# microsoft/fadtk

Hardware: NVIDIA H100
Metric: audio_seconds_embedded_per_second (higher is better)
Workload: dtype f16

## Files before the change

fadtk_b200/csrc/conv_gemm.cuh:

```cuda
#pragma once
#include "sm90.cuh"

namespace fad {

struct ConvGemmParams {
    int taps;
    int cblks;
    int box_w, box_h, box_n;
    int tiles_w, tiles_h;
    int img_groups;
    int n_tiles;
    int H, W, NB, Cout;
    int lo_adds;
    int ld_out, n_valid;
    int relu, pool;
    const float* bias;
    __half* out;
    float* out_f32;
    float* resid;
    int resid_C, resid_res, resid_shift;
};

__device__ __forceinline__ long long window_row_to_token(long long o, int res, int shift) {
    const int lg_nw = 28 - __clz(res);
    const int nw = res >> 3;
    const int in = (int)(o & 63);
    const long long wi = o >> 6;
    const int wx = (int)wi & (nw - 1);
    const int wy = (int)(wi >> lg_nw) & (nw - 1);
    const long long b = wi >> (2 * lg_nw);
    int y = wy * 8 + (in >> 3) + shift, xx = wx * 8 + (in & 7) + shift;
    if (y >= res) y -= res;
    if (xx >= res) xx -= res;
    return (b * res + y) * res + xx;
}

constexpr int kTileM = 128;
constexpr int kBlockK = 64;
constexpr int kConvGemmThreads = 384;
constexpr int kConsumers = 2;
constexpr int kClusterCtas = 2;
constexpr int kChunkSteps = 8;
constexpr float kAccumShrinkPerElement = 1.06e-9f;
constexpr uint32_t kABytes = kTileM * kBlockK * 2;
constexpr uint32_t kEpiRowBytes = 128 * 4;
constexpr uint32_t kEpiBytes = 64 * kEpiRowBytes;
constexpr uint32_t kStagingBytes = 32 * 128;

template <int N_TILE, int WMODE>
__host__ __device__ constexpr uint32_t conv_gemm_stage_bytes() {
    return kABytes + (WMODE == 1 ? 2 : 1) * N_TILE * kBlockK * 2;
}

template <int N_TILE, int STAGES, int WMODE>
__host__ __device__ constexpr uint32_t conv_gemm_smem_bytes() {
    return STAGES * conv_gemm_stage_bytes<N_TILE, WMODE>() + 1024  + 256
         + kConsumers * kEpiBytes;
}

__device__ __forceinline__ uint32_t pack_half2(float a, float b) {
    __half2 h = __floats2half2_rn(a, b);
    return *reinterpret_cast<uint32_t*>(&h);
}
__device__ __forceinline__ float gelu_erf(float x) {
    const float z = fminf(fabsf(x) * 0.70710678118654752f, 4.3f);
    float q = 1.04899843e-04f;
    q = fmaf(q, z, -4.92790774e-04f);
    q = fmaf(q, z, -2.22368206e-03f);
    q = fmaf(q, z, 2.93586859e-02f);
    q = fmaf(q, z, -1.48908889e-01f);
    q = fmaf(q, z, -9.18342944e-01f);
    q = fmaf(q, z, -1.62791250e+00f);
    float e;
    asm("ex2.approx.ftz.f32 %0, %1;" : "=f"(e) : "f"(q * z));
    return 0.5f * x * (1.0f + copysignf(1.0f - e, x));
}

__device__ __forceinline__ float elu_ex2(float x) {
    float e;
    asm("ex2.approx.ftz.f32 %0, %1;" : "=f"(e) : "f"(fminf(x, 0.f) * 1.4426950408889634f));
    const float t = x * fmaf(x, fmaf(x, fmaf(x, 4.16666667e-2f, 1.66666667e-1f), 0.5f), 1.0f);
    return x > 0.f ? x : (x > -0.0625f ? t : e - 1.0f);
}

__device__ __forceinline__ uint32_t hmax2_u32(uint32_t a, uint32_t b) {
    __half2 r = __hmax2(*reinterpret_cast<__half2*>(&a), *reinterpret_cast<__half2*>(&b));
    return *reinterpret_cast<uint32_t*>(&r);
}

template <int N_TILE, int STAGES, int WMODE>
__global__ void __launch_bounds__(kConvGemmThreads, 1)
conv_gemm_kernel(const __grid_constant__ CUtensorMap map_x,
                 const __grid_constant__ CUtensorMap map_w,
                 const ConvGemmParams p)
{
    using namespace sm90;
    static_assert(N_TILE == 128, "one m64n128 accumulator per consumer warpgroup");
    static_assert(WMODE == 0 || WMODE == 1, "WMODE 0: fp16 weights, 1: fp16 hi/lo pair");
    static_assert(kClusterCtas == 2, "the work units below are M-tile pairs");
    constexpr bool SPLIT_W = WMODE == 1;
    constexpr uint32_t kStageBytes = conv_gemm_stage_bytes<N_TILE, WMODE>();
    constexpr int kBRows = (SPLIT_W ? 2 : 1) * N_TILE;
    constexpr int kColsPerThread = N_TILE / 2;
    constexpr int kGroups = kColsPerThread / 32;

    extern __shared__ uint8_t smem_raw[];
    uint8_t* smem = reinterpret_cast<uint8_t*>((reinterpret_cast<uintptr_t>(smem_raw) + 1023) & ~uintptr_t(1023));
    uint64_t* bars = reinterpret_cast<uint64_t*>(smem + STAGES * kStageBytes);
    uint64_t* full = bars;
    uint64_t* empty = bars + STAGES;
    uint8_t* epi = smem + STAGES * kStageBytes + 256;

    const int warp = threadIdx.x >> 5;
    const int lane = threadIdx.x & 31;
    const int ksteps = p.taps * p.cblks;
    const int n_chunks = (ksteps + kChunkSteps - 1) / kChunkSteps;
    const int chunk_len = (ksteps + n_chunks - 1) / n_chunks;
    const int m_tiles = p.img_groups * p.tiles_h * p.tiles_w;
    const int rank = (int)cluster_ctarank();
    const int cluster = (int)blockIdx.x / kClusterCtas;
    const int n_clusters = (int)gridDim.x / kClusterCtas;
    const int total_units = (m_tiles + 1) / 2 * p.n_tiles;

    if (warp == 0 && lane == 0) {
        tma_prefetch_desc(&map_x);
        tma_prefetch_desc(&map_w);
    }
    if (warp == 1 && lane == 0) {
        for (int s = 0; s < STAGES; ++s) { mbar_init(&full[s], 1); mbar_init(&empty[s], kClusterCtas * kConsumers * 4); }
        mbar_fence_init();
    }
    cluster_sync();

    if (warp < 4) {
        setmaxnreg_dec<40>();
        if (warp == 0 && elect_one()) {
            constexpr int kHalfRows = kBRows / kClusterCtas;
            uint8_t* const w_half = smem + kABytes + rank * kHalfRows * 128;
            int s = 0; uint32_t ph = 0;
            for (int unit = cluster; unit < total_units; unit += n_clusters) {
                const int nt = unit % p.n_tiles;
                const int m = min(2 * (unit / p.n_tiles) + rank, m_tiles - 1);
                const int w0 = (m % p.tiles_w) * p.box_w;
                const int h0 = ((m / p.tiles_w) % p.tiles_h) * p.box_h;
                const int n0 = (m / (p.tiles_w * p.tiles_h)) * p.box_n;
                for (int ks = 0; ks < ksteps; ++ks) {
                    const int tap = ks / p.cblks;
                    const int cb = ks - tap * p.cblks;
                    int dh = 0, dw = 0;
                    if (p.taps == 9) { dh = tap / 3 - 1; dw = tap % 3 - 1; }
                    mbar_wait(&empty[s], ph ^ 1);
                    uint8_t* st = smem + s * kStageBytes;
                    mbar_expect_tx(&full[s], kStageBytes);
                    tma_load_4d(st, &map_x, &full[s], cb * kBlockK, w0 + dw, h0 + dh, n0);
                    tma_load_2d_multicast(w_half + s * kStageBytes, &map_w, &full[s], ks * kBlockK,
                                          nt * kBRows + rank * kHalfRows, (1u << kClusterCtas) - 1);
                    if (++s == STAGES) { s = 0; ph ^= 1; }
                }
            }
        }
    } else {
        setmaxnreg_inc<232>();
        const int c = (warp >> 2) - 1;
        const int wg_t = threadIdx.x & 127;
        const int wq = wg_t >> 5;
        const int rr = wg_t & 63;
        const int half = wg_t >> 6;
        const int r = c * 64 + rr;
        const int bw = p.box_w, bh = p.box_h;
        const int pw = r % bw;
        const int phh = (r / bw) % bh;
        const int pn = r / (bw * bh);
        const uint32_t epi_base = smem_u32(epi) + c * kEpiBytes;
        const uint32_t bar_id = 1 + c;
        int s = 0; uint32_t ph = 0;
        const bool plain = p.tiles_w == 1 && p.tiles_h == 1 && bw == 1 && bh == 1;
        auto prefetch_resid = [&](int nt_, int m_) {
            if (p.resid == nullptr || !plain) return;
            const int n_ = m_ * kTileM + r;
            if (n_ >= p.NB) return;
            const long long tok = p.resid_res ? window_row_to_token((long long)n_, p.resid_res, p.resid_shift) : (long long)n_;
            const int c0 = nt_ * N_TILE + half * kColsPerThread;
            for (int cc = c0; cc < c0 + kColsPerThread && cc < p.resid_C; cc += 32)
                asm volatile("prefetch.global.L2 [%0];" :: "l"(p.resid + tok * p.resid_C + cc));
        };
        if (cluster < total_units) prefetch_resid(cluster % p.n_tiles, 2 * (cluster / p.n_tiles) + rank);
        auto load_bias = [&](float4 (&b)[8], int col0) {
            const float4* src = reinterpret_cast<const float4*>(p.bias + col0);
#pragma unroll
            for (int j = 0; j < 8; ++j) b[j] = __ldg(src + j);
        };
        auto release = [&](int st_) {
            __syncwarp();
            if (lane == 0) {
#pragma unroll
                for (int cta = 0; cta < kClusterCtas; ++cta) mbar_arrive_cluster(&empty[st_], cta);
            }
        };

        for (int unit = cluster; unit < total_units; unit += n_clusters) {
            const int nt = unit % p.n_tiles;
            const int m = 2 * (unit / p.n_tiles) + rank;
            if (unit + n_clusters < total_units)
                prefetch_resid((unit + n_clusters) % p.n_tiles, 2 * ((unit + n_clusters) / p.n_tiles) + rank);

            float sum[64], acc[64];
#pragma unroll
            for (int i = 0; i < 64; ++i) sum[i] = 0.f;
            for (int ks0 = 0; ks0 < ksteps; ks0 += chunk_len) {
                const int ks1 = min(ks0 + chunk_len, ksteps);
                const float unshrink = kAccumShrinkPerElement * (float)((ks1 - ks0) * kBlockK * (SPLIT_W && p.lo_adds ? 2 : 1));
                int prev_s = -1;
                for (int ks = ks0; ks < ks1; ++ks) {
                    mbar_wait(&full[s], ph);
                    const uint32_t a_addr = smem_u32(smem + s * kStageBytes);
                    const uint64_t a_desc = kmajor_sw128_desc(a_addr + c * 64 * 128);
                    const uint64_t b_desc = kmajor_sw128_desc(a_addr + kABytes);
                    wgmma_fence();
#pragma unroll
                    for (int k = 0; k < kBlockK / 16; ++k) {
                        wgmma_m64n128k16_f16<0, 0>(acc, a_desc + 2 * k, b_desc + 2 * k, (ks > ks0) || (k > 0));
                        if (SPLIT_W)
                            wgmma_m64n128k16_f16<0, 0>(acc, a_desc + 2 * k, b_desc + 2 * k + (N_TILE * 128 / 16), 1);
                    }
                    wgmma_commit();
                    wgmma_wait<1>();
                    if (prev_s >= 0) release(prev_s);
                    prev_s = s;
                    if (++s == STAGES) { s = 0; ph ^= 1; }
                }
                wgmma_wait<0>();
                fence_regs(acc);
                release(prev_s);
#pragma unroll
                for (int i = 0; i < 64; ++i) sum[i] += fmaf(acc[i], unshrink, acc[i]);
            }

            named_bar_sync(bar_id, 128);
            {
                const int fr = wq * 16 + (lane >> 2);
#pragma unroll
                for (int j = 0; j < 16; ++j) {
#pragma unroll
                    for (int i = 0; i < 2; ++i) {
                        const int row = fr + 8 * i, col = 8 * j + 2 * (lane & 3);
                        const uint32_t addr = epi_base + row * kEpiRowBytes + ((((col >> 2) ^ (row & 7))) << 4) + (col & 3) * 4;
                        sts64(addr, sum[4 * j + 2 * i], sum[4 * j + 2 * i + 1]);
                    }
                }
            }
            named_bar_sync(bar_id, 128);
            float accr[kColsPerThread];
#pragma unroll
            for (int q4 = 0; q4 < kColsPerThread / 4; ++q4) {
                const int ch = half * (kColsPerThread / 4) + q4;
                const uint4 u = lds128(epi_base + rr * kEpiRowBytes + ((ch ^ (rr & 7)) << 4));
                accr[4 * q4 + 0] = __uint_as_float(u.x); accr[4 * q4 + 1] = __uint_as_float(u.y);
                accr[4 * q4 + 2] = __uint_as_float(u.z); accr[4 * q4 + 3] = __uint_as_float(u.w);
            }
            named_bar_sync(bar_id, 128);

            int w, h, n;
            if (plain) { w = 0; h = 0; n = m * kTileM + r; }
            else {
                w = (m % p.tiles_w) * bw + pw;
                h = ((m / p.tiles_w) % p.tiles_h) * bh + phh;
                n = (m / (p.tiles_w * p.tiles_h)) * p.box_n + pn;
            }
            const bool valid = n < p.NB;
            const int ch0 = nt * N_TILE + half * kColsPerThread;
            long long out_off = -1, res_off = -1;
            if (valid && !p.pool) {
                out_off = (long long)((size_t(n) * p.H + h) * p.W + w) * p.ld_out;
                if (p.resid != nullptr)
                    res_off = (p.resid_res ? window_row_to_token((long long)n, p.resid_res, p.resid_shift) : (long long)n)
                              * p.resid_C;
            }
            const uint32_t stg = epi_base + wq * kStagingBytes;
            const uint32_t stg_mine = stg + lane * 128;
            const int sw = lane & 7;
            const int cq = lane & 7, rq = lane >> 3;
            const bool f32_path = p.out_f32 != nullptr || p.resid != nullptr;
            float4 bnext[8];
#pragma unroll
            for (int g = 0; g < kGroups; ++g) {
                float f[32];
                load_bias(bnext, ch0 + g * 32);
#pragma unroll
                for (int j = 0; j < 8; ++j) {
                    const float4 b = bnext[j];
                    f[4 * j + 0] = accr[g * 32 + 4 * j + 0] + b.x;
                    f[4 * j + 1] = accr[g * 32 + 4 * j + 1] + b.y;
                    f[4 * j + 2] = accr[g * 32 + 4 * j + 2] + b.z;
                    f[4 * j + 3] = accr[g * 32 + 4 * j + 3] + b.w;
                }
                if (p.relu == 1) {
#pragma unroll
                    for (int j = 0; j < 32; ++j) f[j] = fmaxf(f[j], 0.0f);
                } else if (p.relu == 2) {
#pragma unroll
                    for (int j = 0; j < 32; ++j) f[j] = gelu_erf(f[j]);
                } else if (p.relu == 3) {
#pragma unroll
                    for (int j = 0; j < 32; ++j) f[j] = elu_ex2(f[j]);
                }
                uint32_t h2[16];
#pragma unroll
                for (int j = 0; j < 16; ++j) h2[j] = pack_half2(f[2 * j], f[2 * j + 1]);

                if (!p.pool) {
                    if (f32_path) {
#pragma unroll
                        for (int j = 0; j < 8; ++j)
                            sts128(stg_mine + ((j ^ sw) << 4), __float_as_uint(f[4 * j]), __float_as_uint(f[4 * j + 1]),
                                   __float_as_uint(f[4 * j + 2]), __float_as_uint(f[4 * j + 3]));
                        __syncwarp();
                        float4 v[8];
#pragma unroll
                        for (int it = 0; it < 8; ++it) {
                            const int rr = it * 4 + rq;
                            const uint4 u = lds128(stg + rr * 128 + ((cq ^ (rr & 7)) << 4));
                            v[it] = make_float4(__uint_as_float(u.x), __uint_as_float(u.y), __uint_as_float(u.z), __uint_as_float(u.w));
                        }
                        const int col = ch0 + g * 32 + cq * 4;
                        if (p.out_f32 != nullptr) {
#pragma unroll
                            for (int it = 0; it < 8; ++it) {
                                const long long off = __shfl_sync(0xffffffffu, out_off, it * 4 + rq);
                                if (off >= 0 && col < p.n_valid) *reinterpret_cast<float4*>(p.out_f32 + off + col) = v[it];
                            }
                        }
                        if (p.resid != nullptr && ch0 + g * 32 < p.resid_C) {
#pragma unroll
                            for (int hf = 0; hf < 2; ++hf) {
                                long long offs[4];
                                float4 xv[4];
#pragma unroll
                                for (int it = 0; it < 4; ++it) {
                                    offs[it] = __shfl_sync(0xffffffffu, res_off, (hf * 4 + it) * 4 + rq);
                                    if (offs[it] >= 0) xv[it] = *reinterpret_cast<const float4*>(p.resid + offs[it] + col);
                                }
#pragma unroll
                                for (int it = 0; it < 4; ++it) {
                                    if (offs[it] >= 0) {
                                        const float4 a = v[hf * 4 + it];
                                        xv[it].x += a.x; xv[it].y += a.y; xv[it].z += a.z; xv[it].w += a.w;
                                        *reinterpret_cast<float4*>(p.resid + offs[it] + col) = xv[it];
                                    }
                                }
                            }
                        }
                        __syncwarp();
                        if (p.out != nullptr && out_off >= 0) {
                            uint4* dst = reinterpret_cast<uint4*>(p.out + out_off + ch0 + g * 32);
#pragma unroll
                            for (int j = 0; j < 4; ++j)
                                if (ch0 + g * 32 + 8 * j < p.n_valid)
                                    dst[j] = make_uint4(h2[4 * j], h2[4 * j + 1], h2[4 * j + 2], h2[4 * j + 3]);
                        }
                    } else if (p.out != nullptr) {
#pragma unroll
                        for (int j = 0; j < 4; ++j)
                            sts128(stg_mine + ((((g & 1) * 4 + j) ^ sw) << 4), h2[4 * j], h2[4 * j + 1], h2[4 * j + 2], h2[4 * j + 3]);
                        if (g & 1) {
                            __syncwarp();
                            const int col = ch0 + (g - 1) * 32 + cq * 8;
#pragma unroll
                            for (int it = 0; it < 8; ++it) {
                                const int rr = it * 4 + rq;
                                const uint4 v = lds128(stg + rr * 128 + ((cq ^ (rr & 7)) << 4));
                                const long long off = __shfl_sync(0xffffffffu, out_off, rr);
                                if (off >= 0 && col < p.n_valid) *reinterpret_cast<uint4*>(p.out + off + col) = v;
                            }
                            __syncwarp();
                        }
                    }
                } else {
#pragma unroll
                    for (int j = 0; j < 16; ++j) {
                        uint32_t o = __shfl_xor_sync(0xffffffffu, h2[j], 1);
                        h2[j] = hmax2_u32(h2[j], o);
                        o = __shfl_xor_sync(0xffffffffu, h2[j], bw);
                        h2[j] = hmax2_u32(h2[j], o);
                    }
                    const int sub = (pw & 1) | ((phh & 1) << 1);
                    uint4 o;
                    o.x = sub == 0 ? h2[0] : sub == 1 ? h2[4] : sub == 2 ? h2[8]  : h2[12];
                    o.y = sub == 0 ? h2[1] : sub == 1 ? h2[5] : sub == 2 ? h2[9]  : h2[13];
                    o.z = sub == 0 ? h2[2] : sub == 1 ? h2[6] : sub == 2 ? h2[10] : h2[14];
                    o.w = sub == 0 ? h2[3] : sub == 1 ? h2[7] : sub == 2 ? h2[11] : h2[15];
                    if (valid) {
                        const size_t pix = (size_t(n) * (p.H >> 1) + (h >> 1)) * (p.W >> 1) + (w >> 1);
                        *reinterpret_cast<uint4*>(p.out + pix * p.Cout + ch0 + g * 32 + sub * 8) = o;
                    }
                }
            }
        }
    }
    cluster_sync();
}

}
```

fadtk_b200/csrc/sm90.cuh:

```cuda
#pragma once
#include <cuda.h>
#include <cuda_fp16.h>
#include <stdint.h>
#include <stdio.h>

namespace sm90 {

__device__ __forceinline__ uint32_t smem_u32(const void* p) {
    return static_cast<uint32_t>(__cvta_generic_to_shared(p));
}
__device__ __forceinline__ uint32_t lane_id() { return threadIdx.x & 31; }

__device__ __forceinline__ bool elect_one() {
    uint32_t pred;
    asm volatile(
        "{\n\t.reg .pred P;\n\t"
        "elect.sync _|P, 0xffffffff;\n\t"
        "selp.u32 %0, 1, 0, P;\n\t}\n"
        : "=r"(pred));
    return pred != 0;
}

template <uint32_t kRegs> __device__ __forceinline__ void setmaxnreg_inc() {
    asm volatile("setmaxnreg.inc.sync.aligned.u32 %0;" ::"n"(kRegs));
}
template <uint32_t kRegs> __device__ __forceinline__ void setmaxnreg_dec() {
    asm volatile("setmaxnreg.dec.sync.aligned.u32 %0;" ::"n"(kRegs));
}

__device__ __forceinline__ void named_bar_sync(uint32_t id, uint32_t count) {
    asm volatile("bar.sync %0, %1;" ::"r"(id), "r"(count) : "memory");
}

__device__ __forceinline__ void sts128(uint32_t addr, uint32_t x, uint32_t y, uint32_t z, uint32_t w) {
    asm volatile("st.shared.v4.b32 [%0], {%1, %2, %3, %4};" ::"r"(addr), "r"(x), "r"(y), "r"(z), "r"(w) : "memory");
}
__device__ __forceinline__ uint4 lds128(uint32_t addr) {
    uint4 v;
    asm volatile("ld.shared.v4.b32 {%0, %1, %2, %3}, [%4];" : "=r"(v.x), "=r"(v.y), "=r"(v.z), "=r"(v.w) : "r"(addr) : "memory");
    return v;
}
__device__ __forceinline__ void sts64(uint32_t addr, float x, float y) {
    asm volatile("st.shared.v2.f32 [%0], {%1, %2};" ::"r"(addr), "f"(x), "f"(y) : "memory");
}

__device__ __forceinline__ void mbar_init(uint64_t* bar, uint32_t count) {
    asm volatile("mbarrier.init.shared::cta.b64 [%0], %1;" ::"r"(smem_u32(bar)), "r"(count));
}
__device__ __forceinline__ void mbar_fence_init() {
    asm volatile("fence.mbarrier_init.release.cluster;" ::: "memory");
}
__device__ __forceinline__ void mbar_expect_tx(uint64_t* bar, uint32_t bytes) {
    asm volatile("mbarrier.arrive.expect_tx.shared::cta.b64 _, [%0], %1;"
                 ::"r"(smem_u32(bar)), "r"(bytes) : "memory");
}
__device__ __forceinline__ void mbar_arrive(uint64_t* bar) {
    asm volatile("mbarrier.arrive.shared::cta.b64 _, [%0];" ::"r"(smem_u32(bar)) : "memory");
}
__device__ __forceinline__ bool mbar_try_wait(uint64_t* bar, uint32_t parity) {
    uint32_t ok;
    asm volatile(
        "{\n\t.reg .pred P;\n\t"
        "mbarrier.try_wait.parity.shared::cta.b64 P, [%1], %2;\n\t"
        "selp.u32 %0, 1, 0, P;\n\t}\n"
        : "=r"(ok) : "r"(smem_u32(bar)), "r"(parity) : "memory");
    return ok != 0;
}
__device__ __forceinline__ bool mbar_try_wait_hint(uint64_t* bar, uint32_t parity, uint32_t ns) {
    uint32_t ok;
    asm volatile(
        "{\n\t.reg .pred P;\n\t"
        "mbarrier.try_wait.parity.shared::cta.b64 P, [%1], %2, %3;\n\t"
        "selp.u32 %0, 1, 0, P;\n\t}\n"
        : "=r"(ok) : "r"(smem_u32(bar)), "r"(parity), "r"(ns) : "memory");
    return ok != 0;
}
__device__ __forceinline__ void mbar_wait(uint64_t* bar, uint32_t parity) {
    if (mbar_try_wait(bar, parity)) return;
    uint32_t spins = 0;
    while (!mbar_try_wait_hint(bar, parity, 2000u)) {
        if (++spins > (1u << 24)) asm volatile("trap;");
    }
}

__device__ __forceinline__ uint32_t cluster_ctarank() {
    uint32_t r;
    asm volatile("mov.u32 %0, %%cluster_ctarank;" : "=r"(r));
    return r;
}
__device__ __forceinline__ void cluster_sync() {
    asm volatile("barrier.cluster.arrive.release;\n\tbarrier.cluster.wait.acquire;" ::: "memory");
}
__device__ __forceinline__ void mbar_arrive_cluster(uint64_t* bar, uint32_t cta) {
    asm volatile(
        "{\n\t.reg .b32 ra;\n\t"
        "mapa.shared::cluster.u32 ra, %0, %1;\n\t"
        "mbarrier.arrive.shared::cluster.b64 _, [ra];\n\t}\n"
        ::"r"(smem_u32(bar)), "r"(cta) : "memory");
}

__device__ __forceinline__ void fence_proxy_async_smem() {
    asm volatile("fence.proxy.async.shared::cta;" ::: "memory");
}

__device__ __forceinline__ void tma_prefetch_desc(const CUtensorMap* m) {
    asm volatile("prefetch.tensormap [%0];" ::"l"(reinterpret_cast<uint64_t>(m)) : "memory");
}
__device__ __forceinline__ void tma_load_2d(void* dst, const CUtensorMap* m, uint64_t* bar,
                                            int c0, int c1) {
    asm volatile(
        "cp.async.bulk.tensor.2d.shared::cluster.global.mbarrier::complete_tx::bytes"
        " [%0], [%1, {%3, %4}], [%2];"
        ::"r"(smem_u32(dst)), "l"(reinterpret_cast<uint64_t>(m)), "r"(smem_u32(bar)),
          "r"(c0), "r"(c1) : "memory");
}
__device__ __forceinline__ void tma_load_2d_multicast(void* dst, const CUtensorMap* m, uint64_t* bar,
                                                      int c0, int c1, uint16_t cta_mask) {
    asm volatile(
        "cp.async.bulk.tensor.2d.shared::cluster.global.mbarrier::complete_tx::bytes.multicast::cluster"
        " [%0], [%1, {%3, %4}], [%2], %5;"
        ::"r"(smem_u32(dst)), "l"(reinterpret_cast<uint64_t>(m)), "r"(smem_u32(bar)),
          "r"(c0), "r"(c1), "h"(cta_mask) : "memory");
}
__device__ __forceinline__ void tma_load_3d(void* dst, const CUtensorMap* m, uint64_t* bar,
                                            int c0, int c1, int c2) {
    asm volatile(
        "cp.async.bulk.tensor.3d.shared::cluster.global.mbarrier::complete_tx::bytes"
        " [%0], [%1, {%3, %4, %5}], [%2];"
        ::"r"(smem_u32(dst)), "l"(reinterpret_cast<uint64_t>(m)), "r"(smem_u32(bar)),
          "r"(c0), "r"(c1), "r"(c2) : "memory");
}
__device__ __forceinline__ void tma_load_4d(void* dst, const CUtensorMap* m, uint64_t* bar,
                                            int c0, int c1, int c2, int c3) {
    asm volatile(
        "cp.async.bulk.tensor.4d.shared::cluster.global.mbarrier::complete_tx::bytes"
        " [%0], [%1, {%3, %4, %5, %6}], [%2];"
        ::"r"(smem_u32(dst)), "l"(reinterpret_cast<uint64_t>(m)), "r"(smem_u32(bar)),
          "r"(c0), "r"(c1), "r"(c2), "r"(c3) : "memory");
}

enum : uint64_t { SWZ_NONE = 0, SWZ_128B = 1, SWZ_64B = 2, SWZ_32B = 3 };

__device__ __forceinline__ uint64_t make_smem_desc(uint32_t saddr, uint32_t lbo_bytes,
                                                   uint32_t sbo_bytes, uint64_t swizzle) {
    return  (uint64_t)((saddr & 0x3FFFF) >> 4)
          | ((uint64_t)(lbo_bytes >> 4) << 16)
          | ((uint64_t)(sbo_bytes >> 4) << 32)
          | (swizzle << 62);
}

__device__ __forceinline__ uint64_t kmajor_sw128_desc(uint32_t saddr) {
    return make_smem_desc(saddr, 16, 1024, SWZ_128B);
}
__device__ __forceinline__ uint64_t mnmajor_sw128_desc(uint32_t saddr, uint32_t lbo_bytes,
                                                       uint32_t sbo_bytes) {
    return make_smem_desc(saddr, lbo_bytes, sbo_bytes, SWZ_128B);
}

__device__ __forceinline__ void wgmma_fence() { asm volatile("wgmma.fence.sync.aligned;" ::: "memory"); }
__device__ __forceinline__ void wgmma_commit() { asm volatile("wgmma.commit_group.sync.aligned;" ::: "memory"); }
template <int N> __device__ __forceinline__ void wgmma_wait() {
    asm volatile("wgmma.wait_group.sync.aligned %0;" ::"n"(N) : "memory");
}
template <int N> __device__ __forceinline__ void fence_regs(float (&d)[N]) {
#pragma unroll
    for (int i = 0; i < N; ++i) asm volatile("" : "+f"(d[i])::"memory");
}

#define FAD_WG_D64                                                                                                 \
    "{%0, %1, %2, %3, %4, %5, %6, %7, %8, %9, %10, %11, %12, %13, %14, %15, "                                    \
    "%16, %17, %18, %19, %20, %21, %22, %23, %24, %25, %26, %27, %28, %29, %30, %31, "                            \
    "%32, %33, %34, %35, %36, %37, %38, %39, %40, %41, %42, %43, %44, %45, %46, %47, "                            \
    "%48, %49, %50, %51, %52, %53, %54, %55, %56, %57, %58, %59, %60, %61, %62, %63}"
#define FAD_WG_OUT64(d)                                                                                            \
    "+f"(d[0]), "+f"(d[1]), "+f"(d[2]), "+f"(d[3]), "+f"(d[4]), "+f"(d[5]), "+f"(d[6]), "+f"(d[7]),                \
    "+f"(d[8]), "+f"(d[9]), "+f"(d[10]), "+f"(d[11]), "+f"(d[12]), "+f"(d[13]), "+f"(d[14]), "+f"(d[15]),          \
    "+f"(d[16]), "+f"(d[17]), "+f"(d[18]), "+f"(d[19]), "+f"(d[20]), "+f"(d[21]), "+f"(d[22]), "+f"(d[23]),        \
    "+f"(d[24]), "+f"(d[25]), "+f"(d[26]), "+f"(d[27]), "+f"(d[28]), "+f"(d[29]), "+f"(d[30]), "+f"(d[31]),        \
    "+f"(d[32]), "+f"(d[33]), "+f"(d[34]), "+f"(d[35]), "+f"(d[36]), "+f"(d[37]), "+f"(d[38]), "+f"(d[39]),        \
    "+f"(d[40]), "+f"(d[41]), "+f"(d[42]), "+f"(d[43]), "+f"(d[44]), "+f"(d[45]), "+f"(d[46]), "+f"(d[47]),        \
    "+f"(d[48]), "+f"(d[49]), "+f"(d[50]), "+f"(d[51]), "+f"(d[52]), "+f"(d[53]), "+f"(d[54]), "+f"(d[55]),        \
    "+f"(d[56]), "+f"(d[57]), "+f"(d[58]), "+f"(d[59]), "+f"(d[60]), "+f"(d[61]), "+f"(d[62]), "+f"(d[63])

template <int TA, int TB>
__device__ __forceinline__ void wgmma_m64n128k16_f16(float (&d)[64], uint64_t a_desc, uint64_t b_desc, uint32_t accumulate) {
    asm volatile(
        "{\n\t.reg .pred p;\n\t"
        "setp.ne.b32 p, %66, 0;\n\t"
        "wgmma.mma_async.sync.aligned.m64n128k16.f32.f16.f16 " FAD_WG_D64 ", %64, %65, p, 1, 1, %67, %68;\n\t}\n"
        : FAD_WG_OUT64(d)
        : "l"(a_desc), "l"(b_desc), "r"(accumulate), "n"(TA), "n"(TB));
}

#define FAD_WG_D32                                                                                                 \
    "{%0, %1, %2, %3, %4, %5, %6, %7, %8, %9, %10, %11, %12, %13, %14, %15, "                                    \
    "%16, %17, %18, %19, %20, %21, %22, %23, %24, %25, %26, %27, %28, %29, %30, %31}"
__device__ __forceinline__ void wgmma_m64n64k16_f16_rs(float (&d)[32], const uint32_t (&a)[4], uint64_t b_desc, uint32_t accumulate) {
    asm volatile(
        "{\n\t.reg .pred p;\n\t"
        "setp.ne.b32 p, %37, 0;\n\t"
        "wgmma.mma_async.sync.aligned.m64n64k16.f32.f16.f16 " FAD_WG_D32 ", {%32, %33, %34, %35}, %36, p, 1, 1, 1;\n\t}\n"
        : "+f"(d[0]), "+f"(d[1]), "+f"(d[2]), "+f"(d[3]), "+f"(d[4]), "+f"(d[5]), "+f"(d[6]), "+f"(d[7]),
          "+f"(d[8]), "+f"(d[9]), "+f"(d[10]), "+f"(d[11]), "+f"(d[12]), "+f"(d[13]), "+f"(d[14]), "+f"(d[15]),
          "+f"(d[16]), "+f"(d[17]), "+f"(d[18]), "+f"(d[19]), "+f"(d[20]), "+f"(d[21]), "+f"(d[22]), "+f"(d[23]),
          "+f"(d[24]), "+f"(d[25]), "+f"(d[26]), "+f"(d[27]), "+f"(d[28]), "+f"(d[29]), "+f"(d[30]), "+f"(d[31])
        : "r"(a[0]), "r"(a[1]), "r"(a[2]), "r"(a[3]), "l"(b_desc), "r"(accumulate));
}

}
```

Before: 173,900.

## Add dedicated epilogue warpgroup to overlap epilogue with next tile's MMA

Result: faster. 179,500 (median of 6 runs) (+3.2%).

```diff
diff --git a/fadtk_b200/csrc/conv_gemm.cuh b/fadtk_b200/csrc/conv_gemm.cuh
--- a/fadtk_b200/csrc/conv_gemm.cuh
+++ b/fadtk_b200/csrc/conv_gemm.cuh
@@ -37,15 +37,19 @@
 
 constexpr int kTileM = 128;
 constexpr int kBlockK = 64;
-constexpr int kConvGemmThreads = 384;
+constexpr int kConvGemmThreads = 512;
 constexpr int kConsumers = 2;
+constexpr int kConsumerRegs = 168;
+constexpr int kEpiRegs = 136;
 constexpr int kClusterCtas = 2;
 constexpr int kChunkSteps = 8;
 constexpr float kAccumShrinkPerElement = 1.06e-9f;
 constexpr uint32_t kABytes = kTileM * kBlockK * 2;
 constexpr uint32_t kEpiRowBytes = 128 * 4;
 constexpr uint32_t kEpiBytes = 64 * kEpiRowBytes;
-constexpr uint32_t kStagingBytes = 32 * 128;
+constexpr uint32_t kBiasBytes = 128 * 4;
+static_assert(40 + kEpiRegs + kConsumers * kConsumerRegs <= 65536 / 128, "register file over-subscribed");
+static_assert(kConsumerRegs > 65536 / kConvGemmThreads, "the consumers raise their register count (setmaxnreg.inc)");
 
 template <int N_TILE, int WMODE>
 __host__ __device__ constexpr uint32_t conv_gemm_stage_bytes() {
@@ -55,32 +59,44 @@
 template <int N_TILE, int STAGES, int WMODE>
 __host__ __device__ constexpr uint32_t conv_gemm_smem_bytes() {
     return STAGES * conv_gemm_stage_bytes<N_TILE, WMODE>() + 1024  + 256
-         + kConsumers * kEpiBytes;
+         + kConsumers * kEpiBytes + 4 * kBiasBytes;
 }
 
 __device__ __forceinline__ uint32_t pack_half2(float a, float b) {
     __half2 h = __floats2half2_rn(a, b);
     return *reinterpret_cast<uint32_t*>(&h);
 }
+template <int N>
+__device__ __forceinline__ void gelu_erf_n(float* x) {
+    float z[N], q[N];
+#pragma unroll
+    for (int i = 0; i < N; ++i) { z[i] = fminf(fabsf(x[i]) * 0.70710678118654752f, 4.3f); q[i] = 1.04899843e-04f; }
+    constexpr float kQ[6] = {-4.92790774e-04f, -2.22368206e-03f, 2.93586859e-02f, -1.48908889e-01f, -9.18342944e-01f,
+                             -1.62791250e+00f};
+#pragma unroll
+    for (int t = 0; t < 6; ++t) {
+#pragma unroll
+        for (int i = 0; i < N; ++i) q[i] = fmaf(q[i], z[i], kQ[t]);
+    }
+#pragma unroll
+    for (int i = 0; i < N; ++i) asm("ex2.approx.ftz.f32 %0, %1;" : "=f"(q[i]) : "f"(q[i] * z[i]));
+#pragma unroll
+    for (int i = 0; i < N; ++i) x[i] = 0.5f * x[i] * (1.0f + copysignf(1.0f - q[i], x[i]));
+}
 __device__ __forceinline__ float gelu_erf(float x) {
-    const float z = fminf(fabsf(x) * 0.70710678118654752f, 4.3f);
-    float q = 1.04899843e-04f;
-    q = fmaf(q, z, -4.92790774e-04f);
-    q = fmaf(q, z, -2.22368206e-03f);
-    q = fmaf(q, z, 2.93586859e-02f);
-    q = fmaf(q, z, -1.48908889e-01f);
-    q = fmaf(q, z, -9.18342944e-01f);
-    q = fmaf(q, z, -1.62791250e+00f);
-    float e;
-    asm("ex2.approx.ftz.f32 %0, %1;" : "=f"(e) : "f"(q * z));
-    return 0.5f * x * (1.0f + copysignf(1.0f - e, x));
-}
-
-__device__ __forceinline__ float elu_ex2(float x) {
-    float e;
-    asm("ex2.approx.ftz.f32 %0, %1;" : "=f"(e) : "f"(fminf(x, 0.f) * 1.4426950408889634f));
-    const float t = x * fmaf(x, fmaf(x, fmaf(x, 4.16666667e-2f, 1.66666667e-1f), 0.5f), 1.0f);
-    return x > 0.f ? x : (x > -0.0625f ? t : e - 1.0f);
+    gelu_erf_n<1>(&x);
+    return x;
+}
+
+template <int N>
+__device__ __forceinline__ void elu_ex2_n(float* x) {
+    float e[N], t[N];
+#pragma unroll
+    for (int i = 0; i < N; ++i) asm("ex2.approx.ftz.f32 %0, %1;" : "=f"(e[i]) : "f"(fminf(x[i], 0.f) * 1.4426950408889634f));
+#pragma unroll
+    for (int i = 0; i < N; ++i) t[i] = x[i] * fmaf(x[i], fmaf(x[i], fmaf(x[i], 4.16666667e-2f, 1.66666667e-1f), 0.5f), 1.0f);
+#pragma unroll
+    for (int i = 0; i < N; ++i) x[i] = x[i] > 0.f ? x[i] : (x[i] > -0.0625f ? t[i] : e[i] - 1.0f);
 }
 
 __device__ __forceinline__ uint32_t hmax2_u32(uint32_t a, uint32_t b) {
@@ -101,14 +117,16 @@
     constexpr bool SPLIT_W = WMODE == 1;
     constexpr uint32_t kStageBytes = conv_gemm_stage_bytes<N_TILE, WMODE>();
     constexpr int kBRows = (SPLIT_W ? 2 : 1) * N_TILE;
-    constexpr int kColsPerThread = N_TILE / 2;
-    constexpr int kGroups = kColsPerThread / 32;
+    constexpr int kGroups = N_TILE / 32;
 
     extern __shared__ uint8_t smem_raw[];
     uint8_t* smem = reinterpret_cast<uint8_t*>((reinterpret_cast<uintptr_t>(smem_raw) + 1023) & ~uintptr_t(1023));
     uint64_t* bars = reinterpret_cast<uint64_t*>(smem + STAGES * kStageBytes);
     uint64_t* full = bars;
     uint64_t* empty = bars + STAGES;
+    uint64_t* epi_full = bars + 2 * STAGES;
+    uint64_t* epi_empty = bars + 2 * STAGES + kConsumers;
+    static_assert((2 * STAGES + 2 * kConsumers) * 8 <= 256, "barriers");
     uint8_t* epi = smem + STAGES * kStageBytes + 256;
 
     const int warp = threadIdx.x >> 5;
@@ -117,8 +135,6 @@
     const int n_chunks = (ksteps + kChunkSteps - 1) / kChunkSteps;
     const int chunk_len = (ksteps + n_chunks - 1) / n_chunks;
     const int m_tiles = p.img_groups * p.tiles_h * p.tiles_w;
-    const int rank = (int)cluster_ctarank();
-    const int cluster = (int)blockIdx.x / kClusterCtas;
     const int n_clusters = (int)gridDim.x / kClusterCtas;
     const int total_units = (m_tiles + 1) / 2 * p.n_tiles;
 
@@ -128,6 +144,7 @@
     }
     if (warp == 1 && lane == 0) {
         for (int s = 0; s < STAGES; ++s) { mbar_init(&full[s], 1); mbar_init(&empty[s], kClusterCtas * kConsumers * 4); }
+        for (int c = 0; c < kConsumers; ++c) { mbar_init(&epi_full[c], 128); mbar_init(&epi_empty[c], 64); }
         mbar_fence_init();
     }
     cluster_sync();
@@ -135,6 +152,8 @@
     if (warp < 4) {
         setmaxnreg_dec<40>();
         if (warp == 0 && elect_one()) {
+            const int rank = (int)cluster_ctarank();
+            const int cluster = (int)cluster_index();
             constexpr int kHalfRows = kBRows / kClusterCtas;
             uint8_t* const w_half = smem + kABytes + rank * kHalfRows * 128;
             int s = 0; uint32_t ph = 0;
@@ -159,37 +178,13 @@
                 }
             }
         }
-    } else {
-        setmaxnreg_inc<232>();
+    } else if (warp < 4 + 4 * kConsumers) {
+        setmaxnreg_inc<kConsumerRegs>();
+        const int cluster = (int)cluster_index();
         const int c = (warp >> 2) - 1;
-        const int wg_t = threadIdx.x & 127;
-        const int wq = wg_t >> 5;
-        const int rr = wg_t & 63;
-        const int half = wg_t >> 6;
-        const int r = c * 64 + rr;
-        const int bw = p.box_w, bh = p.box_h;
-        const int pw = r % bw;
-        const int phh = (r / bw) % bh;
-        const int pn = r / (bw * bh);
+        const int wq = warp & 3;
         const uint32_t epi_base = smem_u32(epi) + c * kEpiBytes;
-        const uint32_t bar_id = 1 + c;
-        int s = 0; uint32_t ph = 0;
-        const bool plain = p.tiles_w == 1 && p.tiles_h == 1 && bw == 1 && bh == 1;
-        auto prefetch_resid = [&](int nt_, int m_) {
-            if (p.resid == nullptr || !plain) return;
-            const int n_ = m_ * kTileM + r;
-            if (n_ >= p.NB) return;
-            const long long tok = p.resid_res ? window_row_to_token((long long)n_, p.resid_res, p.resid_shift) : (long long)n_;
-            const int c0 = nt_ * N_TILE + half * kColsPerThread;
-            for (int cc = c0; cc < c0 + kColsPerThread && cc < p.resid_C; cc += 32)
-                asm volatile("prefetch.global.L2 [%0];" :: "l"(p.resid + tok * p.resid_C + cc));
-        };
-        if (cluster < total_units) prefetch_resid(cluster % p.n_tiles, 2 * (cluster / p.n_tiles) + rank);
-        auto load_bias = [&](float4 (&b)[8], int col0) {
-            const float4* src = reinterpret_cast<const float4*>(p.bias + col0);
-#pragma unroll
-            for (int j = 0; j < 8; ++j) b[j] = __ldg(src + j);
-        };
+        int s = 0; uint32_t ph = 0, eph = 0;
         auto release = [&](int st_) {
             __syncwarp();
             if (lane == 0) {
@@ -199,11 +194,6 @@
         };
 
         for (int unit = cluster; unit < total_units; unit += n_clusters) {
-            const int nt = unit % p.n_tiles;
-            const int m = 2 * (unit / p.n_tiles) + rank;
-            if (unit + n_clusters < total_units)
-                prefetch_resid((unit + n_clusters) % p.n_tiles, 2 * ((unit + n_clusters) / p.n_tiles) + rank);
-
             float sum[64], acc[64];
 #pragma unroll
             for (int i = 0; i < 64; ++i) sum[i] = 0.f;
@@ -236,29 +226,67 @@
                 for (int i = 0; i < 64; ++i) sum[i] += fmaf(acc[i], unshrink, acc[i]);
             }
 
-            named_bar_sync(bar_id, 128);
+            mbar_wait(&epi_empty[c], eph ^ 1);
+            const int fr = wq * 16 + (lane >> 2);
+            const uint32_t x = ((lane & 3) >> 1) ^ (fr & 7);
+            const uint32_t row_base = epi_base + fr * kEpiRowBytes + (lane & 1) * 8;
+#pragma unroll
+            for (int jl = 0; jl < 4; ++jl) {
+                const uint32_t a = row_base + (((2 * jl) ^ x) << 4);
+#pragma unroll
+                for (int jh = 0; jh < 4; ++jh) {
+#pragma unroll
+                    for (int i = 0; i < 2; ++i) {
+                        const int j = 4 * jh + jl;
+                        sts64(a + i * 8 * kEpiRowBytes + jh * 128, sum[4 * j + 2 * i], sum[4 * j + 2 * i + 1]);
+                    }
+                }
+            }
+            mbar_arrive(&epi_full[c]);
+            eph ^= 1;
+        }
+    } else {
+        if constexpr (kEpiRegs > 65536 / kConvGemmThreads) setmaxnreg_inc<kEpiRegs>();
+        else setmaxnreg_dec<kEpiRegs>();
+        const int rank = (int)cluster_ctarank();
+        const int cluster = (int)cluster_index();
+        const int e = warp - 4 - 4 * kConsumers;
+        const int c = e >> 1;
+        const int rr = (e & 1) * 32 + lane;
+        const int r = c * 64 + rr;
+        const int bw = p.box_w, bh = p.box_h;
+        const int pw = r % bw;
+        const int phh = (r / bw) % bh;
+        const int pn = r / (bw * bh);
+        const uint32_t wrows = smem_u32(epi) + c * kEpiBytes + (e & 1) * 32 * kEpiRowBytes;
+        const uint32_t row_mine = wrows + lane * kEpiRowBytes;
+        const uint32_t bias_s = smem_u32(epi) + kConsumers * kEpiBytes + e * kBiasBytes;
+        const int sw = lane & 7;
+        const int cq = lane & 7, rq = lane >> 3;
+        uint32_t eph = 0;
+        const bool plain = p.tiles_w == 1 && p.tiles_h == 1 && bw == 1 && bh == 1;
+        const bool f32_path = p.out_f32 != nullptr || p.resid != nullptr;
+        auto prefetch_resid = [&](int nt_, int m_) {
+            if (p.resid == nullptr || !plain) return;
+            const int n_ = m_ * kTileM + r;
+            if (n_ >= p.NB) return;
+            const long long tok = p.resid_res ? window_row_to_token((long long)n_, p.resid_res, p.resid_shift) : (long long)n_;
+            for (int cc = nt_ * N_TILE; cc < nt_ * N_TILE + N_TILE && cc < p.resid_C; cc += 32)
+                asm volatile("prefetch.global.L2 [%0];" :: "l"(p.resid + tok * p.resid_C + cc));
+        };
+        if (cluster < total_units) prefetch_resid(cluster % p.n_tiles, 2 * (cluster / p.n_tiles) + rank);
+
+        for (int unit = cluster; unit < total_units; unit += n_clusters) {
+            const int nt = unit % p.n_tiles;
+            const int m = 2 * (unit / p.n_tiles) + rank;
+            if (unit + n_clusters < total_units)
+                prefetch_resid((unit + n_clusters) % p.n_tiles, 2 * ((unit + n_clusters) / p.n_tiles) + rank);
+            __syncwarp();
             {
-                const int fr = wq * 16 + (lane >> 2);
-#pragma unroll
-                for (int j = 0; j < 16; ++j) {
-#pragma unroll
-                    for (int i = 0; i < 2; ++i) {
-                        const int row = fr + 8 * i, col = 8 * j + 2 * (lane & 3);
-                        const uint32_t addr = epi_base + row * kEpiRowBytes + ((((col >> 2) ^ (row & 7))) << 4) + (col & 3) * 4;
-                        sts64(addr, sum[4 * j + 2 * i], sum[4 * j + 2 * i + 1]);
-                    }
-                }
-            }
-            named_bar_sync(bar_id, 128);
-            float accr[kColsPerThread];
-#pragma unroll
-            for (int q4 = 0; q4 < kColsPerThread / 4; ++q4) {
-                const int ch = half * (kColsPerThread / 4) + q4;
-                const uint4 u = lds128(epi_base + rr * kEpiRowBytes + ((ch ^ (rr & 7)) << 4));
-                accr[4 * q4 + 0] = __uint_as_float(u.x); accr[4 * q4 + 1] = __uint_as_float(u.y);
-                accr[4 * q4 + 2] = __uint_as_float(u.z); accr[4 * q4 + 3] = __uint_as_float(u.w);
-            }
-            named_bar_sync(bar_id, 128);
+                const float4 b = __ldg(reinterpret_cast<const float4*>(p.bias + nt * N_TILE) + lane);
+                sts128(bias_s + lane * 16, __float_as_uint(b.x), __float_as_uint(b.y), __float_as_uint(b.z), __float_as_uint(b.w));
+            }
+            __syncwarp();
 
             int w, h, n;
             if (plain) { w = 0; h = 0; n = m * kTileM + r; }
@@ -268,7 +296,7 @@
                 n = (m / (p.tiles_w * p.tiles_h)) * p.box_n + pn;
             }
             const bool valid = n < p.NB;
-            const int ch0 = nt * N_TILE + half * kColsPerThread;
+            const int ch0 = nt * N_TILE;
             long long out_off = -1, res_off = -1;
             if (valid && !p.pool) {
                 out_off = (long long)((size_t(n) * p.H + h) * p.W + w) * p.ld_out;
@@ -276,63 +304,64 @@
                     res_off = (p.resid_res ? window_row_to_token((long long)n, p.resid_res, p.resid_shift) : (long long)n)
                               * p.resid_C;
             }
-            const uint32_t stg = epi_base + wq * kStagingBytes;
-            const uint32_t stg_mine = stg + lane * 128;
-            const int sw = lane & 7;
-            const int cq = lane & 7, rq = lane >> 3;
-            const bool f32_path = p.out_f32 != nullptr || p.resid != nullptr;
-            float4 bnext[8];
-#pragma unroll
+
+            mbar_wait(&epi_full[c], eph);
+#pragma unroll 1
             for (int g = 0; g < kGroups; ++g) {
                 float f[32];
-                load_bias(bnext, ch0 + g * 32);
 #pragma unroll
                 for (int j = 0; j < 8; ++j) {
-                    const float4 b = bnext[j];
-                    f[4 * j + 0] = accr[g * 32 + 4 * j + 0] + b.x;
-                    f[4 * j + 1] = accr[g * 32 + 4 * j + 1] + b.y;
-                    f[4 * j + 2] = accr[g * 32 + 4 * j + 2] + b.z;
-                    f[4 * j + 3] = accr[g * 32 + 4 * j + 3] + b.w;
+                    const uint4 u = lds128(row_mine + g * 128 + ((j ^ sw) << 4));
+                    const uint4 b = lds128(bias_s + g * 128 + j * 16);
+                    f[4 * j + 0] = __uint_as_float(u.x) + __uint_as_float(b.x);
+                    f[4 * j + 1] = __uint_as_float(u.y) + __uint_as_float(b.y);
+                    f[4 * j + 2] = __uint_as_float(u.z) + __uint_as_float(b.z);
+                    f[4 * j + 3] = __uint_as_float(u.w) + __uint_as_float(b.w);
                 }
                 if (p.relu == 1) {
 #pragma unroll
                     for (int j = 0; j < 32; ++j) f[j] = fmaxf(f[j], 0.0f);
                 } else if (p.relu == 2) {
 #pragma unroll
-                    for (int j = 0; j < 32; ++j) f[j] = gelu_erf(f[j]);
+                    for (int j = 0; j < 32; j += 8) gelu_erf_n<8>(f + j);
                 } else if (p.relu == 3) {
 #pragma unroll
-                    for (int j = 0; j < 32; ++j) f[j] = elu_ex2(f[j]);
-                }
-                uint32_t h2[16];
-#pragma unroll
-                for (int j = 0; j < 16; ++j) h2[j] = pack_half2(f[2 * j], f[2 * j + 1]);
+                    for (int j = 0; j < 32; j += 8) elu_ex2_n<8>(f + j);
+                }
 
                 if (!p.pool) {
                     if (f32_path) {
+                        if (p.out != nullptr && out_off >= 0) {
+                            uint4* dst = reinterpret_cast<uint4*>(p.out + out_off + ch0 + g * 32);
+#pragma unroll
+                            for (int j = 0; j < 4; ++j)
+                                if (ch0 + g * 32 + 8 * j < p.n_valid)
+                                    dst[j] = make_uint4(pack_half2(f[8 * j], f[8 * j + 1]), pack_half2(f[8 * j + 2], f[8 * j + 3]),
+                                                        pack_half2(f[8 * j + 4], f[8 * j + 5]), pack_half2(f[8 * j + 6], f[8 * j + 7]));
+                        }
 #pragma unroll
                         for (int j = 0; j < 8; ++j)
-                            sts128(stg_mine + ((j ^ sw) << 4), __float_as_uint(f[4 * j]), __float_as_uint(f[4 * j + 1]),
+                            sts128(row_mine + g * 128 + ((j ^ sw) << 4), __float_as_uint(f[4 * j]), __float_as_uint(f[4 * j + 1]),
                                    __float_as_uint(f[4 * j + 2]), __float_as_uint(f[4 * j + 3]));
                         __syncwarp();
-                        float4 v[8];
-#pragma unroll
-                        for (int it = 0; it < 8; ++it) {
-                            const int rr = it * 4 + rq;
-                            const uint4 u = lds128(stg + rr * 128 + ((cq ^ (rr & 7)) << 4));
-                            v[it] = make_float4(__uint_as_float(u.x), __uint_as_float(u.y), __uint_as_float(u.z), __uint_as_float(u.w));
-                        }
                         const int col = ch0 + g * 32 + cq * 4;
-                        if (p.out_f32 != nullptr) {
-#pragma unroll
-                            for (int it = 0; it < 8; ++it) {
-                                const long long off = __shfl_sync(0xffffffffu, out_off, it * 4 + rq);
-                                if (off >= 0 && col < p.n_valid) *reinterpret_cast<float4*>(p.out_f32 + off + col) = v[it];
+#pragma unroll
+                        for (int hf = 0; hf < 2; ++hf) {
+                            float4 v[4];
+#pragma unroll
+                            for (int it = 0; it < 4; ++it) {
+                                const int x = (hf * 4 + it) * 4 + rq;
+                                const uint4 u = lds128(wrows + x * kEpiRowBytes + g * 128 + ((cq ^ (x & 7)) << 4));
+                                v[it] = make_float4(__uint_as_float(u.x), __uint_as_float(u.y), __uint_as_float(u.z), __uint_as_float(u.w));
                             }
-                        }
-                        if (p.resid != nullptr && ch0 + g * 32 < p.resid_C) {
-#pragma unroll
-                            for (int hf = 0; hf < 2; ++hf) {
+                            if (p.out_f32 != nullptr) {
+#pragma unroll
+                                for (int it = 0; it < 4; ++it) {
+                                    const long long off = __shfl_sync(0xffffffffu, out_off, (hf * 4 + it) * 4 + rq);
+                                    if (off >= 0 && col < p.n_valid) *reinterpret_cast<float4*>(p.out_f32 + off + col) = v[it];
+                                }
+                            }
+                            if (p.resid != nullptr && ch0 + g * 32 < p.resid_C) {
                                 long long offs[4];
                                 float4 xv[4];
 #pragma unroll
@@ -343,39 +372,36 @@
 #pragma unroll
                                 for (int it = 0; it < 4; ++it) {
                                     if (offs[it] >= 0) {
-                                        const float4 a = v[hf * 4 + it];
+                                        const float4 a = v[it];
                                         xv[it].x += a.x; xv[it].y += a.y; xv[it].z += a.z; xv[it].w += a.w;
                                         *reinterpret_cast<float4*>(p.resid + offs[it] + col) = xv[it];
                                     }
                                 }
                             }
                         }
-                        __syncwarp();
-                        if (p.out != nullptr && out_off >= 0) {
-                            uint4* dst = reinterpret_cast<uint4*>(p.out + out_off + ch0 + g * 32);
-#pragma unroll
-                            for (int j = 0; j < 4; ++j)
-                                if (ch0 + g * 32 + 8 * j < p.n_valid)
-                                    dst[j] = make_uint4(h2[4 * j], h2[4 * j + 1], h2[4 * j + 2], h2[4 * j + 3]);
-                        }
                     } else if (p.out != nullptr) {
+                        const int seg = (g & ~1) * 128;
 #pragma unroll
                         for (int j = 0; j < 4; ++j)
-                            sts128(stg_mine + ((((g & 1) * 4 + j) ^ sw) << 4), h2[4 * j], h2[4 * j + 1], h2[4 * j + 2], h2[4 * j + 3]);
+                            sts128(row_mine + seg + ((((g & 1) * 4 + j) ^ sw) << 4),
+                                   pack_half2(f[8 * j], f[8 * j + 1]), pack_half2(f[8 * j + 2], f[8 * j + 3]),
+                                   pack_half2(f[8 * j + 4], f[8 * j + 5]), pack_half2(f[8 * j + 6], f[8 * j + 7]));
                         if (g & 1) {
                             __syncwarp();
                             const int col = ch0 + (g - 1) * 32 + cq * 8;
 #pragma unroll
                             for (int it = 0; it < 8; ++it) {
-                                const int rr = it * 4 + rq;
-                                const uint4 v = lds128(stg + rr * 128 + ((cq ^ (rr & 7)) << 4));
-                                const long long off = __shfl_sync(0xffffffffu, out_off, rr);
+                                const int x = it * 4 + rq;
+                                const uint4 v = lds128(wrows + x * kEpiRowBytes + seg + ((cq ^ (x & 7)) << 4));
+                                const long long off = __shfl_sync(0xffffffffu, out_off, x);
                                 if (off >= 0 && col < p.n_valid) *reinterpret_cast<uint4*>(p.out + off + col) = v;
                             }
-                            __syncwarp();
                         }
                     }
                 } else {
+                    uint32_t h2[16];
+#pragma unroll
+                    for (int j = 0; j < 16; ++j) h2[j] = pack_half2(f[2 * j], f[2 * j + 1]);
 #pragma unroll
                     for (int j = 0; j < 16; ++j) {
                         uint32_t o = __shfl_xor_sync(0xffffffffu, h2[j], 1);
@@ -395,6 +421,8 @@
                     }
                 }
             }
+            mbar_arrive(&epi_empty[c]);
+            eph ^= 1;
         }
     }
     cluster_sync();
diff --git a/fadtk_b200/csrc/sm90.cuh b/fadtk_b200/csrc/sm90.cuh
--- a/fadtk_b200/csrc/sm90.cuh
+++ b/fadtk_b200/csrc/sm90.cuh
@@ -86,6 +86,11 @@
 __device__ __forceinline__ uint32_t cluster_ctarank() {
     uint32_t r;
     asm volatile("mov.u32 %0, %%cluster_ctarank;" : "=r"(r));
+    return r;
+}
+__device__ __forceinline__ uint32_t cluster_index() {
+    uint32_t r;
+    asm volatile("mov.u32 %0, %%clusterid.x;" : "=r"(r));
     return r;
 }
 __device__ __forceinline__ void cluster_sync() {
```
